# ChristodoulosPappas/IPLS-Java-API

Measured on AMD Instinct MI355X. Metric: aggregated-gradient GB/s (device-resident), 32 peers×4M doubles/partition, higher is better.
Workload: dtype f64

## Files before the change

### ipls-java-api_amd/csrc/engine.hip

```cpp
#include <hip/hip_runtime.h>

#include <algorithm>
#include <atomic>
#include <cstdarg>
#include <cstdio>
#include <cstdlib>
#include <cstring>
#include <deque>
#include <map>
#include <memory>
#include <mutex>
#include <new>
#include <set>
#include <string>
#include <thread>
#include <type_traits>
#include <vector>

#include "../../include/ipls_agg.h"
#include "ipls_kernels.hpp"
#include "javaser.hpp"
#include "engine.hpp"
#include "operand.hpp"
#include "pubsub_host.hpp"
#include "reduce_plan.hpp"

using namespace ipls;
using namespace ipls::reduceplan;
namespace op = ipls::operand;

namespace {

thread_local std::string g_tls_err;

constexpr int64_t kAlignElems = 32;
constexpr int kRingSlots = 4;
constexpr int kStageSlots = 3;

int64_t align_up(int64_t x, int64_t a) { return (x + a - 1) / a * a; }

struct PinnedSlot {
  void* host = nullptr;
  size_t cap = 0;
  hipEvent_t ev = nullptr;
  bool pending = false;
};

}

struct ipls_stage {
  hipStream_t copy[2] = {};
  int n_copy = 0;
  static constexpr int kMaxSlots = 4;
  PinnedSlot slot[kMaxSlots];
  int n_slot = 0;
  void* d = nullptr;
  size_t d_cap = 0;
  hipEvent_t landed[2] = {};
  hipEvent_t ready = nullptr;
  hipEvent_t free_ev = nullptr;
  bool free_pending = false;
};

struct ipls_dev {
  std::mutex mu;
  std::string err;
  int device = 0;
  hipStream_t stream = nullptr;

  int64_t model_size = 0;
  int P = 0;
  int64_t chunk = 0;
  int secure = 0;
  std::vector<int64_t> len, flat_off;
  int64_t max_len = 0, flat_total = 0;
  int p_lo = 0;
  int64_t flat_base = 0;

  double* arena = nullptr;
  int64_t arena_elems = 0;
  std::vector<int64_t> agg_off, rep_off, w_off, fut_off;
  std::vector<uint8_t> agg_zero, rep_zero, fut_zero;

  PinnedSlot ring[kRingSlots];
  void* d_table[kRingSlots] = {};
  size_t d_table_cap[kRingSlots] = {};
  int ring_next = 0;
  std::vector<unsigned char> last_table;
  int last_slot = -1;

  std::mutex stage_mu;
  std::vector<ipls_stage*> stage_all, stage_idle;
  void* d_scratch = nullptr;
  size_t scratch_bytes = 0;
  hipEvent_t copy_ev = nullptr;
  static constexpr int kCopyThreads = 4;
  hipStream_t copy_stream[kCopyThreads] = {};
  hipEvent_t ingest_ev = nullptr;
  std::vector<hipEvent_t> msg_ev;
  struct StageSlot {
    void* d = nullptr;
    size_t cap = 0;
    hipEvent_t free_ev = nullptr;
    bool pending = false;
  };
  StageSlot stage[2];
  int stage_next = 0;
  struct Pending {
    std::vector<const void*> bufs;
    Fmt fmt = kFmtF64;
  };
  std::vector<Pending> pend;
  std::vector<int> pend_keys;
  int pending_n = 0;
  int coalesce = 32;
  struct Batch {
    uint64_t max_ticket;
    hipEvent_t ev;
  };
  static constexpr int kMaxBatches = 64;
  std::deque<Batch> batches;
  std::vector<hipEvent_t> ev_free;
  uint64_t ticket_next = 1, ticket_done = 0, launched_upto = 0;

  unsigned long long* d_sum = nullptr;
  double* d_cnt = nullptr;
  unsigned long long* d_gbuf = nullptr;
  unsigned long long* d_merge = nullptr;
  int64_t merge_cap = 0;
  struct OtherRep {
    unsigned long long* d = nullptr;
    int64_t n = 0;
    int32_t received = 0;
  };
  std::map<std::pair<int, int32_t>, OtherRep> other;
  int64_t gbuf_len = 0;
  ipls_launch_info last_launch{};
};

namespace {

int fail(ipls_dev* h, int code, const char* fmt, ...) {
  char buf[512];
  va_list ap;
  va_start(ap, fmt);
  vsnprintf(buf, sizeof buf, fmt, ap);
  va_end(ap);
  if (h) h->err = buf;
  g_tls_err = buf;
  return code;
}

int not_taken(ipls_dev* h, const op::Refusal& why) { return why.code ? fail(h, why.code, "%s", why.text) : IPLS_OK; }

int flush_pending(ipls_dev* h);

#define IPLS_LOCK(h)                            \
  std::lock_guard<std::mutex> lk_(h->mu);       \
  if (int rc_ = flush_pending(h)) return rc_

#define HIP_TRY(h, expr)                                                                \
  do {                                                                                  \
    hipError_t e_ = (expr);                                                             \
// ... 355 lines not shown
  static constexpr int G = G_, R = R_, MAP = MAP_, BS = BS_, SEQF = SEQF_;
};
template <bool BE_IN, bool BE_OUT, int START, bool FIN = false>
ipls_launch_info launch_reduce_v(int64_t maxL, int n_parts, hipStream_t st, const unsigned long long* const* bufs,
                                 const PartDesc* parts, int k, int secure = 0, const double* cnts = nullptr) {
  constexpr int R = big_r(BE_IN, START), SEQF = big_seqf(BE_IN, START);
  constexpr int RM = mid_r(BE_IN, START), SEQFM = mid_seqf(BE_IN, START);
  const ReducePlan p = plan_reduce(BE_IN, START, FIN, maxL, n_parts);
  const dim3 grid((unsigned)p.grid);
  auto run = [&](auto t) {
    typedef decltype(t) T;
    if constexpr (FIN)
      hipLaunchKernelGGL((k_round<BE_IN, START, T::G, T::R, T::MAP, T::BS, T::SEQF>), grid, dim3(T::BS), 0, st, bufs,
                         parts, k, (int)p.tpp, n_parts, secure, cnts);
    else
      hipLaunchKernelGGL((k_reduce<BE_IN, BE_OUT, START, T::G, T::R, true, T::MAP, T::BS, T::SEQF>), grid,
                         dim3(T::BS), 0, st, bufs, parts, k, (int)p.tpp, n_parts);
  };
  switch (p.shape) {
    case IPLS_SHAPE_HALF:
      if constexpr (half_allowed(START, FIN)) {
        if (p.map == 3) run(Tiles<kBigG, kHalfR, 3, kHalfBS, 0>{});
        else run(Tiles<kBigG, kHalfR, kBigMap, kHalfBS, 0>{});
      }
      break;
    case IPLS_SHAPE_BIG:
      if (p.map == 3) run(Tiles<kBigG, R, 3, kBigBS, SEQF>{});
      else if (p.map == 2) run(Tiles<kBigG, R, 2, kBigBS, SEQF>{});
      else run(Tiles<kBigG, R, kBigMap, kBigBS, SEQF>{});
      break;
    case IPLS_SHAPE_MID:
      if (p.map == 3) run(Tiles<kBigG, RM, 3, kMidBS, SEQFM>{});
      else run(Tiles<kBigG, RM, kBigMap, kMidBS, SEQFM>{});
      break;
    default: run(Tiles<kSmallG, kSmallR, kSmallMap, kSmallBS, 0>{});
  }
  return launch_info(p, BE_IN, BE_OUT, START);
}

ipls_launch_info launch_reduce(bool be_in, bool be_out, int start, int64_t maxL, int n_parts, hipStream_t st,
                               const unsigned long long* const* bufs, const PartDesc* parts, int k) {
  return with_fold(be_in, be_out, start, [&](auto i, auto o, auto s) {
    return launch_reduce_v<decltype(i)::value, decltype(o)::value, decltype(s)::value>(maxL, n_parts, st, bufs, parts, k);
  });
}

ipls_launch_info launch_reduce_fin(bool be_in, int start, int secure, int64_t maxL, int n_parts, hipStream_t st,
                                   const unsigned long long* const* bufs, const PartDesc* parts, int k,
                                   double* cnts) {
  return with_bool(be_in, [&](auto bi) {
    return with_start_za(start, [&](auto s) {
      constexpr bool BI = decltype(bi)::value;
      constexpr int ST = decltype(s)::value;
      hipLaunchKernelGGL((k_round_counts<BI, ST>), dim3(n_parts), dim3(64), 0, st, bufs, parts, k, n_parts, cnts);
      return launch_reduce_v<BI, false, ST, true>(maxL, n_parts, st, bufs, parts, k, secure, cnts);
    });
  });
}

void launch_reduce_scalar(bool be_in, bool be_out, int start, const ReducePlan& p, hipStream_t st,
                          const unsigned long long* const* bufs, const PartDesc* parts, int k) {
  with_fold(be_in, be_out, start, [&](auto bi, auto bo, auto s) {
    hipLaunchKernelGGL((k_reduce_scalar<decltype(bi)::value, decltype(bo)::value, decltype(s)::value>),
                       dim3((unsigned)p.grid), dim3(kBlock), 0, st, bufs, parts, k, (int)p.tpp, p.tile);
  });
}

template <class S>
ipls_launch_info launch_reduce_narrow(bool be_out, int start, bool vec, int64_t maxL, int n_parts, hipStream_t st,
                                      const typename S::elem* const* bufs, const PartDesc* parts, int k) {
  constexpr NarrowShape K = narrow_shape(sizeof(typename S::elem));
  const ReducePlan p = plan_reduce_narrow(sizeof(typename S::elem), false, vec, maxL, n_parts);
  const dim3 grid((unsigned)p.grid);
  with_bool(be_out, [&](auto bo) {
    with_start(start, [&](auto s) {
      auto run = [&](auto map, auto v) {
        constexpr bool V = decltype(v)::value;
        hipLaunchKernelGGL((k_reduce_narrow<S, decltype(bo)::value, decltype(s)::value, K.r, K.bs, decltype(map)::value,
                                            V, (V ? K.pf : 0), K.e>),
                           grid, dim3(K.bs), 0, st, bufs, parts, k, (int)p.tpp, n_parts);
      };
      if (!vec) run(Int<0>{}, std::false_type{});
      else if (p.map == 3) run(Int<3>{}, std::true_type{});
      else run(Int<0>{}, std::true_type{});
    });
  });
  return launch_info(p, false, be_out, start);
}

template <class S, class A>
ipls_launch_info launch_round_narrow(int start, int secure, int64_t maxL, int n_parts, hipStream_t st,
                                     const typename S::elem* const* bufs, const PartDesc* parts, int k,
                                     double* cnts) {
  constexpr NarrowShape K = narrow_shape(sizeof(typename S::elem));
  const ReducePlan p = plan_reduce_narrow(sizeof(typename S::elem), true, true, maxL, n_parts);
  with_start_za(start, [&](auto s) {
    constexpr int ST = decltype(s)::value;
    hipLaunchKernelGGL((k_round_counts_narrow<S, ST>), dim3(n_parts), dim3(64), 0, st, bufs, parts, k, n_parts, cnts);
    hipLaunchKernelGGL((k_round_narrow<S, A, ST, K.r, K.bs, K.pf>), dim3((unsigned)p.grid), dim3(K.bs), 0, st, bufs,
                       parts, k, (int)p.tpp, n_parts, p.map, secure, (const double*)cnts);
  });
  return launch_info(p, false, false, start);
}

struct FinOut {
  unsigned long long* avg;
  Fmt fmt = kFmtF64;
};

constexpr int kFold1NarrowR = 4;
constexpr unsigned kFold1NarrowGrid = 2048;

int reduce_dev(ipls_dev* h, int p_first, int n_parts, const void* const* bufs, int k, Fmt fmt_in,
               int start_mode, int target, void* const* ext_dst = nullptr, bool be_out = false,
               const FinOut* fin = nullptr, bool host_src = false, const int64_t* lens = nullptr,
               bool arrival = false) {
  const bool be_in = fmt_in == kFmtBE, tr_in = fmt_trainer(fmt_in);
  auto len_of = [&](int q) -> int64_t { return lens ? lens[q] : h->len[p_first + q]; };
  auto dst_of = [&](int q) -> unsigned long long* {
    if (fin) return (unsigned long long*)(h->arena + h->w_off[p_first + q]);
    return ext_dst ? (unsigned long long*)ext_dst[q]
                   : (unsigned long long*)(h->arena + target_off(h, p_first + q, target));
  };
  if (k <= 0 && !fin) {
    if (start_mode == IPLS_START_ZERO) {
      for (int q = 0; q < n_parts; ++q) {
        uint8_t* f = ext_dst ? nullptr : zero_flag(h, p_first + q, target);
        if (f) *f = 1;
        else HIP_TRY(h, hipMemsetAsync(dst_of(q), 0, (size_t)len_of(q) * 8, h->stream));
      }
    }
    return IPLS_OK;
  }
  int start = start_mode;
  if (start_mode == IPLS_START_ACCUM && !ext_dst) {
    int nz = 0;
    for (int q = 0; q < n_parts; ++q) {
      uint8_t* f = zero_flag(h, p_first + q, target);
      nz += (f && *f) ? 1 : 0;
    }
    if (nz == n_parts) start = IPLS_START_ZERO;
    else if (nz) {
      for (int q = 0; q < n_parts; ++q) {
        int rc = materialize(h, p_first + q, target);
        if (rc) return rc;
      }
    }
  }
  if (!fin && !tr_in && n_parts == 1 && k == 1 && bufs[0]) {
    unsigned long long* d0 = dst_of(0);
    const int64_t L = len_of(0);
// ... 24 lines not shown
          hipLaunchKernelGGL((k_fold1_narrow<S, decltype(st)::value, kFold1NarrowR>), dim3(blocks), dim3(kBlock), 0,
                             h->stream, d0, s0, L);
        });
      });
      HIP_TRY(h, hipGetLastError());
      h->last_launch = launch_info(fmt_size(fmt_in) == 4 ? IPLS_KERNEL_FOLD1_F32 : IPLS_KERNEL_FOLD1_H16, 0, kBlock,
                                   kFold1NarrowR, 1, 0, blocks, false, false, start);
      if (!ext_dst)
        if (uint8_t* f = zero_flag(h, p_first, target)) *f = 0;
      return IPLS_OK;
    }
  }
  bool aligned16 = true;
  int64_t maxL = 0;
  for (int q = 0; q < n_parts; ++q) maxL = std::max(maxL, len_of(q));
  for (int64_t i = 0; i < (int64_t)n_parts * k; ++i) {
    if (!bufs[i]) return fail(h, IPLS_E_INVAL, "bucket pointer %lld is NULL", (long long)i);
    uintptr_t a = (uintptr_t)bufs[i];
    if (a & (uintptr_t)(fmt_size(fmt_in) - 1))
      return fail(h, IPLS_E_INVAL, "bucket %lld not %d-byte aligned", (long long)i, fmt_size(fmt_in));
    if (a & 15) aligned16 = false;
  }
  const size_t desc_bytes = sizeof(PartDesc) * n_parts;
  const size_t bytes = desc_bytes + sizeof(void*) * (size_t)n_parts * k;
  std::vector<unsigned char> tbl(bytes);
  PartDesc* pd = (PartDesc*)tbl.data();
  for (int q = 0; q < n_parts; ++q) {
    const int p = p_first + q;
    pd[q].len = len_of(q);
    pd[q].dst = dst_of(q);
    pd[q].init = pd[q].dst;
    pd[q].rep = nullptr;
    pd[q].avg = nullptr;
    if (fin) {
      pd[q].init = (const unsigned long long*)(h->arena + h->agg_off[p]);
      if (!h->rep_zero[p]) pd[q].rep = (const unsigned long long*)(h->arena + h->rep_off[p]);
      if (fin->avg)
        pd[q].avg = (unsigned long long*)((char*)fin->avg +
                                          (h->flat_off[p] - h->flat_off[p_first]) * (int64_t)fmt_size(fin->fmt));
    }
    if (!pd[q].dst) return fail(h, IPLS_E_INVAL, "destination %d is NULL", q);
    if ((uintptr_t)pd[q].dst & 7) return fail(h, IPLS_E_INVAL, "destination %d not 8-byte aligned", q);
    if ((uintptr_t)pd[q].dst & 15) aligned16 = false;
  }
  if (k > 0) std::memcpy(tbl.data() + desc_bytes, bufs, sizeof(void*) * (size_t)n_parts * k);
  void* dtab = nullptr;
  int rc = upload_table(h, tbl.data(), bytes, &dtab);
  if (rc) return rc;
  const PartDesc* dparts = (const PartDesc*)dtab;
  auto dbufs = (const unsigned long long* const*)((char*)dtab + desc_bytes);
  if (fin) {
    if (!aligned16 || (fin->avg && tr_in != fmt_trainer(fin->fmt)))
      return fail(h, IPLS_E_INVAL, "fused round needs 16-B aligned buckets and averages of the buckets' family");
    if (tr_in) {
      h->last_launch = with_narrow(fmt_in, [&](auto s) {
        typedef decltype(s) S;
        return with_narrow(fin->avg ? fin->fmt : fmt_in, [&](auto a) {
          return launch_round_narrow<S, decltype(a)>(start, h->secure, maxL, n_parts, h->stream,
                                                     (const typename S::elem* const*)dbufs, dparts, k, h->d_cnt);
        });
      });
    } else {
      h->last_launch = launch_reduce_fin(be_in, start, h->secure, maxL, n_parts, h->stream, dbufs, dparts, k, h->d_cnt);
    }
    HIP_TRY(h, hipGetLastError());
    for (int q = p_first; q < p_first + n_parts; ++q) h->agg_zero[q] = h->rep_zero[q] = 1;
    return IPLS_OK;
  }
  if (tr_in) {
    h->last_launch = with_narrow(fmt_in, [&](auto s) {
      typedef decltype(s) S;
      return launch_reduce_narrow<S>(be_out, start, aligned16, maxL, n_parts, h->stream,
                                     (const typename S::elem* const*)dbufs, dparts, k);
    });
  } else if (aligned16) {
    h->last_launch = launch_reduce(be_in, be_out, start, maxL, n_parts, h->stream, dbufs, dparts, k);
  } else {
    const ReducePlan p = plan_reduce_scalar(maxL, n_parts);
    launch_reduce_scalar(be_in, be_out, start, p, h->stream, dbufs, dparts, k);
    h->last_launch = launch_info(p, be_in, be_out, start);
  }
  HIP_TRY(h, hipGetLastError());
  if (!ext_dst)
    for (int q = 0; q < n_parts; ++q) {
      uint8_t* f = zero_flag(h, p_first + q, target);
      if (f) *f = 0;
    }
  return IPLS_OK;
}

int partition_geometry(const ipls_agg_cfg* c, std::vector<int64_t>& len, std::vector<int64_t>& off,
                       int64_t& chunk, std::string& why) {
  const int P = c->n_partitions;
  len.resize(P);
  off.resize(P);
  if (c->model_size > 0) {
    chunk = ref_chunk(c->model_size, P);
    for (int i = 0; i < P; ++i) {
      int64_t L = ((int64_t)(i + 1) * chunk > c->model_size) ? c->model_size - (int64_t)i * chunk + 1
                                                             : chunk + 1;
      if (L < 1) {
        char b[160];
        snprintf(b, sizeof b, "partition %d length %lld < 1 (%s)", i, (long long)L,
                 L < 0 ? "NegativeArraySizeException, IPLS.java:1863"
                       : "ArrayIndexOutOfBoundsException, IPLS.java:1894");
        why = b;
        return L < 0 ? IPLS_E_NEGSIZE : IPLS_E_RANGE;
      }
      len[i] = L;
      off[i] = (int64_t)i * chunk;
    }
  } else {
    if (c->bucket_len < 1) {
      why = "bucket_len must be >= 1 when model_size == 0";
      return IPLS_E_INVAL;
    }
// ... 159 lines not shown
    lk.lock();
    return fail(h, IPLS_E_DEVICE, "hipStreamSynchronize failed: %s", hipGetErrorString(e));
  }
  return IPLS_OK;
}

int dev_wait(ipls_dev* h, uint64_t ticket) {
  if (!h) return fail(nullptr, IPLS_E_INVAL, "null handle");
  std::unique_lock<std::mutex> lk(h->mu);
  if (ticket >= h->ticket_next) return fail(h, IPLS_E_INVAL, "ticket %llu was never issued", (unsigned long long)ticket);
  if (ticket <= h->ticket_done) return IPLS_OK;
  if (ticket > h->launched_upto)
    if (int rc = flush_pending(h)) return rc;
  hipEvent_t ev = nullptr;
  uint64_t covered = 0;
  for (const auto& b : h->batches)
    if (b.max_ticket >= ticket) {
      ev = b.ev;
      covered = b.max_ticket;
      break;
    }
  if (!ev) return IPLS_OK;
  lk.unlock();
  const hipError_t e = hipEventSynchronize(ev);
  lk.lock();
  if (e != hipSuccess) {
    (void)hipGetLastError();
    return fail(h, IPLS_E_DEVICE, "hipEventSynchronize failed: %s", hipGetErrorString(e));
  }
  while (!h->batches.empty() && h->batches.front().max_ticket <= covered) {
    h->ev_free.push_back(h->batches.front().ev);
    h->batches.pop_front();
  }
  h->ticket_done = std::max(h->ticket_done, covered);
  return IPLS_OK;
}

int dev_flush(ipls_dev* h) {
  if (!h) return fail(nullptr, IPLS_E_INVAL, "null handle");
  IPLS_LOCK(h);
  return IPLS_OK;
}

int dev_set_coalesce(ipls_dev* h, int max_group) {
  if (!h) return fail(nullptr, IPLS_E_INVAL, "null handle");
  IPLS_LOCK(h);
  h->coalesce = std::max(1, max_group);
  return IPLS_OK;
}

namespace {

int end_batch(ipls_dev* h) {
  hipEvent_t ev;
  if (!h->ev_free.empty()) {
    ev = h->ev_free.back();
    h->ev_free.pop_back();
  } else {
    HIP_TRY(h, hipEventCreateWithFlags(&ev, hipEventDisableTiming));
  }
  HIP_TRY(h, hipEventRecord(ev, h->stream));
  h->batches.push_back({h->ticket_next - 1, ev});
  h->launched_upto = h->ticket_next - 1;
  while ((int)h->batches.size() > ipls_dev::kMaxBatches) {
    const ipls_dev::Batch b = h->batches.front();
    HIP_TRY(h, hipEventSynchronize(b.ev));
    h->batches.pop_front();
    h->ev_free.push_back(b.ev);
    h->ticket_done = std::max(h->ticket_done, b.max_ticket);
  }
  return IPLS_OK;
}

int flush_pending(ipls_dev* h) {
  if (h->pend_keys.empty()) return IPLS_OK;
  HIP_TRY(h, dev_use(h->device));
  int rc = IPLS_OK;
  std::vector<int>& keys = h->pend_keys;
  std::sort(keys.begin(), keys.end());
  std::vector<const void*> tab;
  for (size_t i = 0; i < keys.size() && !rc;) {
    const int key = keys[i], target = key / h->P, p0 = key % h->P;
    const ipls_dev::Pending& q0 = h->pend[key];
    const size_t k = q0.bufs.size();
    size_t j = i + 1;
    int n = 1;
    while (j < keys.size() && keys[j] == key + n && keys[j] / h->P == target && h->pend[keys[j]].bufs.size() == k &&
           h->pend[keys[j]].fmt == q0.fmt) {
      ++n;
      ++j;
    }
    tab.clear();
    for (size_t t = i; t < j; ++t) tab.insert(tab.end(), h->pend[keys[t]].bufs.begin(), h->pend[keys[t]].bufs.end());
    rc = reduce_dev(h, p0, n, tab.data(), (int)k, q0.fmt, IPLS_START_ACCUM, target);
    i = j;
  }
  for (int key : keys) h->pend[key].bufs.clear();
  keys.clear();
  h->pending_n = 0;
  if (rc) return rc;
  return end_batch(h);
}

}

int dev_reduce_batch(ipls_dev* h, int p_first, int n_parts, const void* const* bufs, int k,
                          int src_kind, int start_mode, int target) {
  if (!h) return fail(nullptr, IPLS_E_INVAL, "null handle");
  IPLS_LOCK(h);
  if (n_parts <= 0 || p_first < 0 || p_first + n_parts > h->P)
    return fail(h, IPLS_E_RANGE, "partitions [%d,%d) out of range [0,%d)", p_first, p_first + n_parts, h->P);
  if (src_kind != IPLS_DEV_F64 && src_kind != IPLS_DEV_BE && !kind_trainer_dev(src_kind))
    return fail(h, IPLS_E_INVAL, "reduce_batch takes device buckets (DEV_F64/DEV_BE/DEV_F32/DEV_F16/DEV_BF16)");
  if (start_mode < IPLS_START_ACCUM || start_mode > IPLS_START_FIRST) return fail(h, IPLS_E_INVAL, "bad start mode");
  if (target_off(h, 0, target) < 0) return fail(h, IPLS_E_INVAL, "bad target %d", target);
  if (k < 0 || (k > 0 && !bufs)) return fail(h, IPLS_E_INVAL, "bad bucket list");
  HIP_TRY(h, dev_use(h->device));
  return reduce_dev(h, p_first, n_parts, bufs, k, kind_fmt(src_kind), start_mode, target);
}

int dev_accumulate(ipls_dev* h, int p, int target, const void* src, int64_t n, int src_kind) {
  if (!h) return fail(nullptr, IPLS_E_INVAL, "null handle");
  IPLS_LOCK(h);
  if (int rc = check_part(h, p)) return rc;
  if (target_off(h, p, target) < 0) return fail(h, IPLS_E_INVAL, "bad target %d", target);
  const int64_t L = h->len[p];
  op::Resolved v;
  if (op::resolve(op::kAccumulate, src, n, src_kind, L, &v) != op::kTake) return not_taken(h, v.why);
  HIP_TRY(h, dev_use(h->device));
  const size_t bytes = (size_t)L * fmt_size(v.fmt);
  const void* dptr = v.ptr;
  if (v.host) {
    void* alias = nullptr;
    if (v.from == op::kRaw && !fmt_trainer(v.fmt) && op::zero_copy_arrival(v.ptr, bytes) && is_pinned_host(v.ptr, &alias) &&
        alias) {
      const void* bl[1] = {alias};
      if (int rc = reduce_dev(h, p, 1, bl, 1, v.fmt, IPLS_START_ACCUM, target, nullptr, false, nullptr, true)) return rc;
      HIP_TRY(h, hipStreamSynchronize(h->stream));
      return IPLS_OK;
    }
    if (int rc = stage_bucket(h, v.ptr, bytes, &dptr)) return rc;
  }
  const void* bl[1] = {dptr};
  if (int rc = reduce_dev(h, p, 1, bl, 1, v.fmt, IPLS_START_ACCUM, target, nullptr, false, nullptr, false, nullptr,
                          true))
    return rc;
  return v.host ? release_stage(h) : IPLS_OK;
}

int dev_accumulate_async(ipls_dev* h, int p, int target, const void* src, int64_t n, int src_kind,
                              uint64_t* ticket) {
  if (!h || !ticket) return fail(h, IPLS_E_INVAL, "null argument");
  op::Resolved v;
  if (src && (op::kDev & op::bit(src_kind))) {
    std::lock_guard<std::mutex> lk(h->mu);
    if (int rc = check_part(h, p)) return rc;
    if (target_off(h, p, target) < 0) return fail(h, IPLS_E_INVAL, "bad target %d", target);
    if (op::resolve(op::kAccumulateAsync, src, n, src_kind, h->len[p], &v) != op::kTake) return not_taken(h, v.why);
    const Fmt fmt = v.fmt;
    const int qt = target == IPLS_TGT_WADDR ? IPLS_TGT_WEIGHTS : target;
    if (h->pend.empty()) h->pend.resize((size_t)5 * h->P);
    ipls_dev::Pending& q = h->pend[(size_t)qt * h->P + p];
    if (!q.bufs.empty() && q.fmt != fmt)
      if (int rc = flush_pending(h)) return rc;
    if (q.bufs.empty()) h->pend_keys.push_back(qt * h->P + p);
    q.fmt = fmt;
    q.bufs.push_back(src);
    ++h->pending_n;
    *ticket = h->ticket_next++;
    if ((int)q.bufs.size() >= 2 * h->coalesce || h->pending_n >= h->coalesce * (int)h->pend_keys.size())
      return flush_pending(h);
    return IPLS_OK;
  }
  void* alias = nullptr;
  const bool host = op::kHostD & op::bit(src_kind);
  if (!src || !host || !op::zero_copy_queued(src) || !is_pinned_host(src, &alias) || !alias) {
    int rc = dev_accumulate(h, p, target, src, n, src_kind);
    std::lock_guard<std::mutex> lk(h->mu);
    *ticket = h->ticket_done;
    return rc;
  }
  IPLS_LOCK(h);
  if (int rc = check_part(h, p)) return rc;
  if (target_off(h, p, target) < 0) return fail(h, IPLS_E_INVAL, "bad target %d", target);
  if (op::resolve(op::kAccumulateAsync, src, n, src_kind, h->len[p], &v) != op::kTake) return not_taken(h, v.why);
  HIP_TRY(h, dev_use(h->device));
  const void* bl[1] = {alias};
  if (int rc = reduce_dev(h, p, 1, bl, 1, v.fmt, IPLS_START_ACCUM, target, nullptr, false, nullptr, true)) return rc;
  *ticket = h->ticket_next++;
  return end_batch(h);
}

int dev_accumulate_range(ipls_dev* h, int p, int target, const void* src, int64_t off, int64_t n, int src_kind,
                         uint64_t* ticket) {
  if (!h || !ticket || !src) return fail(h, IPLS_E_INVAL, "null argument");
  IPLS_LOCK(h);
  if (int rc = check_part(h, p)) return rc;
  if (target_off(h, p, target) < 0) return fail(h, IPLS_E_INVAL, "bad target %d", target);
  const int64_t L = h->len[p];
  op::Resolved v;
  if (op::resolve(op::kAccumulateRange, src, n, src_kind, L, &v) != op::kTake) return not_taken(h, v.why);
  if (off < 0 || n < 0 || off > L || n > L - off)
    return fail(h, IPLS_E_RANGE, "range [%lld, %lld) outside partition %d of length %lld", (long long)off,
                (long long)(off + n), p, (long long)L);
  if ((off & 1) || !op::zero_copy_queued(src))
    return fail(h, IPLS_E_INVAL, "a ranged fold needs an even start and 16-B aligned bytes");
  void* alias = nullptr;
  if (!is_pinned_host(src, &alias) || !alias)
    return fail(h, IPLS_E_INVAL, "a ranged fold reads pinned host memory (ipls_host_alloc)");
  if (n == 0) {
    *ticket = h->ticket_done;
    return IPLS_OK;
  }
  HIP_TRY(h, dev_use(h->device));
  if (int rc = materialize(h, p, target)) return rc;
  unsigned long long* d0 = (unsigned long long*)(h->arena + target_off(h, p, target)) + off;
  const auto* s0 = (const unsigned long long*)alias;
  const unsigned blocks = std::max(1u, std::min<unsigned>(blocks_for(n >> 1, kBlock * 4), 128u));
// ... 510 lines not shown
                       (const FinDesc*)dtab, h->arena, tpp);
  HIP_TRY(h, hipGetLastError());
  for (int q = p0; q < p0 + np; ++q) h->agg_zero[q] = h->rep_zero[q] = 1;
  return IPLS_OK;
}

static int divide_table(ipls_dev* h, int p0, int np, const DivDesc** dtab, int* tpp) {
  std::vector<DivDesc> dd(np);
  int64_t maxn = 0;
  for (int q = 0; q < np; ++q) {
    const int p = p0 + q;
    dd[q] = DivDesc{h->len[p], h->w_off[p], h->flat_off[p] - h->flat_off[p0]};
    maxn = std::max(maxn, h->len[p] - 1);
  }
  *tpp = (int)((std::max<int64_t>(maxn, 0) + kDivTile - 1) / kDivTile);
  if (*tpp == 0) return IPLS_OK;
  void* d = nullptr;
  if (int rc = upload_table(h, dd.data(), dd.size() * sizeof(DivDesc), &d)) return rc;
  *dtab = (const DivDesc*)d;
  return IPLS_OK;
}

static int divide_range(ipls_dev* h, int p0, int np, unsigned long long* d_out, bool be) {
  const DivDesc* dtab = nullptr;
  int tpp = 0;
  if (int rc = divide_table(h, p0, np, &dtab, &tpp)) return rc;
  if (tpp == 0) return IPLS_OK;
  with_bool(be, [&](auto b) {
    with_bool(h->secure != 0, [&](auto sec) {
      hipLaunchKernelGGL((k_divide<decltype(b)::value, decltype(sec)::value>), dim3((unsigned)tpp * np), dim3(kBlock),
                         0, h->stream, dtab, (const double*)h->arena, d_out, tpp);
    });
  });
  HIP_TRY(h, hipGetLastError());
  return IPLS_OK;
}

static int divide_range_narrow(ipls_dev* h, int p0, int np, void* d_out, Fmt fmt) {
  const DivDesc* dtab = nullptr;
  int tpp = 0;
  if (int rc = divide_table(h, p0, np, &dtab, &tpp)) return rc;
  if (tpp == 0) return IPLS_OK;
  with_narrow(fmt, [&](auto s) {
    typedef decltype(s) S;
    with_bool(h->secure != 0, [&](auto sec) {
      hipLaunchKernelGGL((k_divide_narrow<S, decltype(sec)::value>), dim3((unsigned)tpp * np), dim3(kBlock), 0,
                         h->stream, dtab, (const double*)h->arena, (typename S::elem*)d_out, tpp);
    });
  });
  HIP_TRY(h, hipGetLastError());
  return IPLS_OK;
}

int dev_finalize(ipls_dev* h, int p, void* sum_out, int sum_kind, double* avg_out) {
  if (!h) return fail(nullptr, IPLS_E_INVAL, "null handle");
  IPLS_LOCK(h);
  int p0 = p, np = 1;
  if (p == IPLS_ALL_PARTITIONS) {
    p0 = 0;
    np = h->P;
    if (sum_out || avg_out) return fail(h, IPLS_E_INVAL, "host outputs need a single partition");
  } else if (int rc = check_part(h, p)) {
    return rc;
  }
  if (sum_out && sum_kind != IPLS_HOST_F64 && sum_kind != IPLS_HOST_BE)
    return fail(h, IPLS_E_INVAL, "sum_kind must be HOST_F64 or HOST_BE");
  HIP_TRY(h, dev_use(h->device));
  if (int rc = finalize_range(h, p0, np)) return rc;

  if (np == 1 && (sum_out || avg_out)) {
    const int64_t L = h->len[p0];
    const double* w = h->arena + h->w_off[p0];
    if (sum_out) {
      if (sum_kind == IPLS_HOST_F64) {
        if (int rc = d2h(h, sum_out, w, (size_t)L * 8)) return rc;
      } else if (sum_kind == IPLS_HOST_BE) {
        if (int rc = be_to_host(h, sum_out, w, L)) return rc;
      } else {
        return fail(h, IPLS_E_INVAL, "sum_kind must be HOST_F64 or HOST_BE");
      }
    }
    if (avg_out && L > 1) {
      if (int rc = ensure_scratch(h, (size_t)L * 8)) return rc;
      if (int rc = divide_range(h, p0, 1, (unsigned long long*)h->d_scratch, false)) return rc;
      if (int rc = d2h(h, avg_out, h->d_scratch, (size_t)(L - 1) * 8)) return rc;
    }
  }
  return IPLS_OK;
}

int dev_finalize_chunked(ipls_dev* h, int p, int sum_kind, int64_t chunk, ipls_chunk_sink sink, void* ctx) {
  if (!h || !sink) return fail_nl(h, IPLS_E_INVAL, "null argument");
  if (chunk < 2 || (chunk & 1))
    return fail_nl(h, IPLS_E_INVAL, "chunk of %lld values: even and >= 2", (long long)chunk);
  if (p < 0 || p >= h->P) return fail_nl(h, IPLS_E_RANGE, "partition %d out of range [0,%d)", p, h->P);
  if (sum_kind != IPLS_HOST_F64 && sum_kind != IPLS_HOST_BE)
    return fail_nl(h, IPLS_E_INVAL, "sum_kind must be HOST_F64 or HOST_BE");
  const int64_t L = h->len[p];
  HIP_TRY_NL(h, dev_use(h->device));
  const int64_t c = std::min(chunk, L);
  ipls_stage* st = nullptr;
  if (int rc = stage_acquire(h, (size_t)L * 8, (size_t)c * 8, &st)) return rc;
  int rc = IPLS_OK;
  {
    std::lock_guard<std::mutex> lk(h->mu);
    rc = flush_pending(h);
    if (!rc) rc = finalize_range(h, p, 1);
    if (!rc) {
      const unsigned long long* w = (const unsigned long long*)(h->arena + h->w_off[p]);
      hipError_t e;
      if (sum_kind == IPLS_HOST_BE) {
        launch_bswap(h->stream, w, (unsigned long long*)st->d, L);
        e = hipGetLastError();
      } else {
        e = hipMemcpyAsync(st->d, w, (size_t)L * 8, hipMemcpyDeviceToDevice, h->stream);
      }
      if (e == hipSuccess) e = hipEventRecord(st->ready, h->stream);
      if (e != hipSuccess) {
        (void)hipGetLastError();
        rc = fail(h, IPLS_E_DEVICE, "W snapshot: %s", hipGetErrorString(e));
      }
    }
  }
  if (rc) {
    (void)hipStreamSynchronize(h->stream);
    (void)hipGetLastError();
    stage_release(h, st);
    return rc;
  }
  return stage_deliver(h, st, L, c, 0, sink, ctx, " (the round is consumed)");
}

int dev_set_weights(ipls_dev* h, int p, const void* src, int64_t n, int src_kind) {
  if (!h || !src) return fail(h, IPLS_E_INVAL, "null argument");
  IPLS_LOCK(h);
  if (int rc = check_part(h, p)) return rc;
  const int64_t L = h->len[p];
  op::Resolved v;
  if (op::resolve(op::kSetWeights, src, n, src_kind, L, &v) != op::kTake) return not_taken(h, v.why);
  HIP_TRY(h, dev_use(h->device));
  const int64_t m = v.from == op::kFrame ? L : v.n;
  double* w = h->arena + h->w_off[p];
  const void* d = v.ptr;
  if (v.host) {
    if (v.fmt == kFmtF64) return stage_h2d(h, w, v.ptr, (size_t)m * 8);
    if (int rc = to_scratch(h, v.ptr, (size_t)m * 8)) return rc;
    d = h->d_scratch;
  } else if (v.fmt == kFmtF64) {
    HIP_TRY(h, hipMemcpyAsync(w, v.ptr, (size_t)m * 8, hipMemcpyDeviceToDevice, h->stream));
    return IPLS_OK;
  }
  launch_bswap(h->stream, (const unsigned long long*)d, (unsigned long long*)w, m);
  HIP_TRY(h, hipGetLastError());
  return IPLS_OK;
}

static int flat_to_device(ipls_dev* h, const op::SrcView& v, const unsigned long long** d) {
  *d = (const unsigned long long*)v.ptr;
  if (!v.host) return IPLS_OK;
  if (int rc = to_scratch(h, v.ptr, (size_t)v.n * fmt_size(v.fmt))) return rc;
// ... 380 lines not shown
  hipError_t e = hipGetLastError();
  if (e != hipSuccess) return fail(nullptr, IPLS_E_DEVICE, "k_synth launch: %s", hipGetErrorString(e));
  return IPLS_OK;
}

int ipls_checksum_dev(const void* src, int64_t n, int src_kind, uint64_t* out, void* stream) {
  if (!out || n < 0 || (n > 0 && !src)) return fail(nullptr, IPLS_E_INVAL, "bad argument");
  if (n == 0) {
    *out = 0;
    return IPLS_OK;
  }
  hipStream_t st = (hipStream_t)stream;
  unsigned long long* d = nullptr;
  if (hipMallocAsync((void**)&d, 8, st) != hipSuccess) {
    (void)hipGetLastError();
    return fail(nullptr, IPLS_E_NOMEM, "hipMallocAsync failed");
  }
  hipMemsetAsync(d, 0, 8, st);
  const dim3 g(std::max(1u, std::min<unsigned>(blocks_for(n, kBlock * 8), 2048)));
  if (src_kind == IPLS_DEV_BE)
    hipLaunchKernelGGL(k_checksum<true>, g, dim3(kBlock), 0, st, (const unsigned long long*)src, n, d);
  else
    hipLaunchKernelGGL(k_checksum<false>, g, dim3(kBlock), 0, st, (const unsigned long long*)src, n, d);
  unsigned long long v = 0;
  hipError_t e = hipGetLastError();
  if (e == hipSuccess) e = hipMemcpyAsync(&v, d, 8, hipMemcpyDeviceToHost, st);
  if (e == hipSuccess) e = hipStreamSynchronize(st);
  hipFreeAsync(d, st);
  if (e != hipSuccess) return fail(nullptr, IPLS_E_DEVICE, "checksum: %s", hipGetErrorString(e));
  *out = v;
  return IPLS_OK;
}

int dev_reduce_batch_out(ipls_dev* h, int p_first, int n_parts, const void* const* bufs, int k, int src_kind,
                              int start_mode, void* const* dst, int dst_kind) {
  if (!h) return fail(nullptr, IPLS_E_INVAL, "null handle");
  IPLS_LOCK(h);
  if (n_parts <= 0 || p_first < 0 || p_first + n_parts > h->P)
    return fail(h, IPLS_E_RANGE, "partitions [%d,%d) out of range [0,%d)", p_first, p_first + n_parts, h->P);
  if (src_kind != IPLS_DEV_F64 && src_kind != IPLS_DEV_BE && !kind_trainer_dev(src_kind))
    return fail(h, IPLS_E_INVAL, "reduce_batch_out takes device buckets (DEV_F64/DEV_BE/DEV_F32/DEV_F16/DEV_BF16)");
  if (dst_kind != IPLS_DEV_F64 && dst_kind != IPLS_DEV_BE)
    return fail(h, IPLS_E_INVAL, "reduce_batch_out writes device buffers (DEV_F64/DEV_BE)");
  if (start_mode < IPLS_START_ACCUM || start_mode > IPLS_START_FIRST) return fail(h, IPLS_E_INVAL, "bad start mode");
  if (!dst || k < 0 || (k > 0 && !bufs)) return fail(h, IPLS_E_INVAL, "bad bucket/destination list");
  HIP_TRY(h, dev_use(h->device));
  return reduce_dev(h, p_first, n_parts, bufs, k, kind_fmt(src_kind), start_mode, IPLS_TGT_AGG, dst,
                    dst_kind == IPLS_DEV_BE);
}

int dev_aggregate_round(ipls_dev* h, int p_first, int n_parts, const void* const* bufs, int k, int src_kind,
                             void* avg_out, int avg_kind) {
  if (!h) return fail(nullptr, IPLS_E_INVAL, "null handle");
  IPLS_LOCK(h);
  if (n_parts <= 0 || p_first < 0 || p_first + n_parts > h->P)
    return fail(h, IPLS_E_RANGE, "partitions [%d,%d) out of range [0,%d)", p_first, p_first + n_parts, h->P);
  if (src_kind != IPLS_DEV_F64 && src_kind != IPLS_DEV_BE && !kind_trainer_dev(src_kind))
    return fail(h, IPLS_E_INVAL, "aggregate_round takes device buckets (DEV_F64/DEV_BE/DEV_F32/DEV_F16/DEV_BF16)");
  const Fmt fmt_in = kind_fmt(src_kind);
  const bool tr_in = fmt_trainer(fmt_in);
  const bool tr_avg = avg_out && kind_trainer(avg_kind);
  const Fmt fmt_avg = tr_avg ? kind_fmt(avg_kind) : kFmtF64;
  if (avg_out && !tr_avg && avg_kind != IPLS_DEV_F64 && avg_kind != IPLS_HOST_F64)
    return fail(h, IPLS_E_INVAL, "avg_kind must be DEV_F64, HOST_F64 or a DEV/HOST F32, F16 or BF16 kind");
  if (k < 0 || (k > 0 && !bufs)) return fail(h, IPLS_E_INVAL, "bad bucket list");
  if (tr_in)
    for (int64_t i = 0; i < (int64_t)n_parts * k; ++i)
      if (!bufs[i] || ((uintptr_t)bufs[i] & (uintptr_t)(fmt_size(fmt_in) - 1)))
        return fail(h, IPLS_E_INVAL, "bucket %lld NULL or not %d-byte aligned", (long long)i, fmt_size(fmt_in));
  HIP_TRY(h, dev_use(h->device));
  const int p_last = p_first + n_parts - 1;
  const int64_t n_avg = h->flat_off[p_last] + h->len[p_last] - 1 - h->flat_off[p_first];
  unsigned long long* d_avg = nullptr;
  if (tr_avg && n_avg > 0) {
    if ((uintptr_t)avg_out & (uintptr_t)(fmt_size(fmt_avg) - 1))
      return fail(h, IPLS_E_INVAL, "output not %d-byte aligned", fmt_size(fmt_avg));
    if (kind_trainer_dev(avg_kind)) {
      d_avg = (unsigned long long*)avg_out;
    } else {
      if (int rc = ensure_scratch(h, (size_t)n_avg * fmt_size(fmt_avg))) return rc;
      d_avg = (unsigned long long*)h->d_scratch;
    }
  } else if (avg_out && n_avg > 0) {
    if (avg_kind == IPLS_DEV_F64) {
      if ((uintptr_t)avg_out & 7) return fail(h, IPLS_E_INVAL, "device output not 8-byte aligned");
      d_avg = (unsigned long long*)avg_out;
    } else {
      if (int rc = ensure_scratch(h, (size_t)n_avg * 8)) return rc;
      d_avg = (unsigned long long*)h->d_scratch;
    }
  }
  bool aligned16 = true;
  for (int64_t i = 0; i < (int64_t)n_parts * k; ++i) aligned16 = aligned16 && !((uintptr_t)bufs[i] & 15);
  if (aligned16 && (tr_in ? (!avg_out || tr_avg) : !tr_avg)) {
    FinOut fo{d_avg, fmt_avg};
    if (int rc = reduce_dev(h, p_first, n_parts, bufs, k, fmt_in, IPLS_START_ACCUM, IPLS_TGT_AGG,
                            nullptr, false, &fo))
      return rc;
  } else {
    if (int rc = reduce_dev(h, p_first, n_parts, bufs, k, fmt_in, IPLS_START_ACCUM, IPLS_TGT_AGG)) return rc;
    if (int rc = finalize_range(h, p_first, n_parts)) return rc;
    if (d_avg) {
      if (tr_avg) {
        if (int rc = divide_range_narrow(h, p_first, n_parts, d_avg, fmt_avg)) return rc;
      } else if (int rc = divide_range(h, p_first, n_parts, d_avg, false)) {
        return rc;
      }
    }
  }
  if (d_avg && kind_trainer_host(avg_kind)) return d2h(h, avg_out, d_avg, (size_t)n_avg * fmt_size(fmt_avg));
  if (d_avg && avg_kind == IPLS_HOST_F64) return d2h(h, avg_out, d_avg, (size_t)n_avg * 8);
  return IPLS_OK;
}

namespace {

int ingest_copy_threads() {
  static const int n = [] {
    const char* e = std::getenv("IPLS_INGEST_COPY_THREADS");
    const int v = e ? std::atoi(e) : 2;
    return std::max(1, std::min(v, (int)ipls_dev::kCopyThreads));
  }();
  return n;
}

}

int dev_ingest_pubsub(ipls_dev* h, int target, const uint8_t* const* msgs, const int64_t* lens, int n_msgs,
                           int layers, const int32_t* parts, int32_t* status) {
  if (!h) return fail(nullptr, IPLS_E_INVAL, "null handle");
  IPLS_LOCK(h);
  if (n_msgs < 0 || (n_msgs > 0 && (!msgs || !lens))) return fail(h, IPLS_E_INVAL, "bad message list");
  if (layers < 1 || layers > 2) return fail(h, IPLS_E_INVAL, "layers must be 1 or 2");
  if (target_off(h, 0, target) < 0) return fail(h, IPLS_E_INVAL, "bad target %d", target);
  if (n_msgs == 0) return 0;
  HIP_TRY(h, dev_use(h->device));

  std::vector<int32_t> st(n_msgs, 0), post(n_msgs, 0), route(n_msgs, -1);
  std::vector<int64_t> dc(n_msgs, 0), dc2(n_msgs, 0);
  std::vector<uint8_t> decode(n_msgs, 0);
  for (int i = 0; i < n_msgs; ++i) {
    const pubsub::Pre pre = pubsub::precheck(msgs[i], lens[i], layers);
    if (pre.status) { st[i] = pre.status; continue; }
    dc[i] = pre.dc;
    dc2[i] = pre.dc2;
    decode[i] = 1;
    if (pre.n == 0) { post[i] = 1; continue; }
// ... 894 lines not shown
```

Before: 7139.

## Fuse pending queue fold into finalize round and skip count kernel when unused

Adds a close_range path that folds only the pending queues for the target partitions and, when buffers are aligned, runs them through the fused reduce-plus-finalize-plus-average kernel. Finalize no longer needs separate flush, finalize and divide passes. Ticket accounting now tracks per-queue first tickets so that partial flushes only mark completed work as launched. The count kernel is skipped when no average is requested. This adds complexity to batch and ticket bookkeeping, and dev_aggregate_round now flushes the pending queues first when given explicit buckets.

```diff
diff --git a/ipls-java-api_amd/csrc/engine.hip b/ipls-java-api_amd/csrc/engine.hip
--- a/ipls-java-api_amd/csrc/engine.hip
+++ b/ipls-java-api_amd/csrc/engine.hip
@@ -24,6 +24,7 @@
 #include "operand.hpp"
 #include "pubsub_host.hpp"
 #include "reduce_plan.hpp"
+#include "ticket_rule.hpp"
 
 using namespace ipls;
 using namespace ipls::reduceplan;
@@ -109,6 +110,7 @@
   struct Pending {
     std::vector<const void*> bufs;
     Fmt fmt = kFmtF64;
+    uint64_t first_ticket = 0;
   };
   std::vector<Pending> pend;
   std::vector<int> pend_keys;
@@ -570,7 +572,8 @@
     return with_start_za(start, [&](auto s) {
       constexpr bool BI = decltype(bi)::value;
       constexpr int ST = decltype(s)::value;
-      hipLaunchKernelGGL((k_round_counts<BI, ST>), dim3(n_parts), dim3(64), 0, st, bufs, parts, k, n_parts, cnts);
+      if (cnts)
+        hipLaunchKernelGGL((k_round_counts<BI, ST>), dim3(n_parts), dim3(64), 0, st, bufs, parts, k, n_parts, cnts);
       return launch_reduce_v<BI, false, ST, true>(maxL, n_parts, st, bufs, parts, k, secure, cnts);
     });
   });
@@ -614,7 +617,8 @@
   const ReducePlan p = plan_reduce_narrow(sizeof(typename S::elem), true, true, maxL, n_parts);
   with_start_za(start, [&](auto s) {
     constexpr int ST = decltype(s)::value;
-    hipLaunchKernelGGL((k_round_counts_narrow<S, ST>), dim3(n_parts), dim3(64), 0, st, bufs, parts, k, n_parts, cnts);
+    if (cnts)
+      hipLaunchKernelGGL((k_round_counts_narrow<S, ST>), dim3(n_parts), dim3(64), 0, st, bufs, parts, k, n_parts, cnts);
     hipLaunchKernelGGL((k_round_narrow<S, A, ST, K.r, K.bs, K.pf>), dim3((unsigned)p.grid), dim3(K.bs), 0, st, bufs,
                        parts, k, (int)p.tpp, n_parts, p.map, secure, (const double*)cnts);
   });
@@ -745,16 +749,17 @@
   if (fin) {
     if (!aligned16 || (fin->avg && tr_in != fmt_trainer(fin->fmt)))
       return fail(h, IPLS_E_INVAL, "fused round needs 16-B aligned buckets and averages of the buckets' family");
+    double* const cnts = fin->avg ? h->d_cnt : nullptr;
     if (tr_in) {
       h->last_launch = with_narrow(fmt_in, [&](auto s) {
         typedef decltype(s) S;
         return with_narrow(fin->avg ? fin->fmt : fmt_in, [&](auto a) {
           return launch_round_narrow<S, decltype(a)>(start, h->secure, maxL, n_parts, h->stream,
-                                                     (const typename S::elem* const*)dbufs, dparts, k, h->d_cnt);
+                                                     (const typename S::elem* const*)dbufs, dparts, k, cnts);
         });
       });
     } else {
-      h->last_launch = launch_reduce_fin(be_in, start, h->secure, maxL, n_parts, h->stream, dbufs, dparts, k, h->d_cnt);
+      h->last_launch = launch_reduce_fin(be_in, start, h->secure, maxL, n_parts, h->stream, dbufs, dparts, k, cnts);
     }
     HIP_TRY(h, hipGetLastError());
     for (int q = p_first; q < p_first + n_parts; ++q) h->agg_zero[q] = h->rep_zero[q] = 1;
@@ -1020,6 +1025,10 @@
 namespace {
 
 int end_batch(ipls_dev* h) {
+  std::vector<uint64_t> first_queued;
+  for (int key : h->pend_keys) first_queued.push_back(h->pend[key].first_ticket);
+  const uint64_t upto = tickets::launched_upto(h->ticket_next, first_queued.data(), first_queued.size());
+  if (upto == h->launched_upto) return IPLS_OK;
   hipEvent_t ev;
   if (!h->ev_free.empty()) {
     ev = h->ev_free.back();
@@ -1028,8 +1037,8 @@
     HIP_TRY(h, hipEventCreateWithFlags(&ev, hipEventDisableTiming));
   }
   HIP_TRY(h, hipEventRecord(ev, h->stream));
-  h->batches.push_back({h->ticket_next - 1, ev});
-  h->launched_upto = h->ticket_next - 1;
+  h->batches.push_back({upto, ev});
+  h->launched_upto = upto;
   while ((int)h->batches.size() > ipls_dev::kMaxBatches) {
     const ipls_dev::Batch b = h->batches.front();
     HIP_TRY(h, hipEventSynchronize(b.ev));
@@ -1040,20 +1049,17 @@
   return IPLS_OK;
 }
 
-int flush_pending(ipls_dev* h) {
-  if (h->pend_keys.empty()) return IPLS_OK;
-  HIP_TRY(h, dev_use(h->device));
+int fold_queues(ipls_dev* h, const std::vector<int>& keys, size_t i, size_t end) {
   int rc = IPLS_OK;
-  std::vector<int>& keys = h->pend_keys;
-  std::sort(keys.begin(), keys.end());
   std::vector<const void*> tab;
-  for (size_t i = 0; i < keys.size() && !rc;) {
+  const size_t first = i;
+  while (i < end && !rc) {
     const int key = keys[i], target = key / h->P, p0 = key % h->P;
     const ipls_dev::Pending& q0 = h->pend[key];
     const size_t k = q0.bufs.size();
     size_t j = i + 1;
     int n = 1;
-    while (j < keys.size() && keys[j] == key + n && keys[j] / h->P == target && h->pend[keys[j]].bufs.size() == k &&
+    while (j < end && keys[j] == key + n && keys[j] / h->P == target && h->pend[keys[j]].bufs.size() == k &&
            h->pend[keys[j]].fmt == q0.fmt) {
       ++n;
       ++j;
@@ -1063,9 +1069,21 @@
     rc = reduce_dev(h, p0, n, tab.data(), (int)k, q0.fmt, IPLS_START_ACCUM, target);
     i = j;
   }
-  for (int key : keys) h->pend[key].bufs.clear();
+  for (size_t t = first; t < end; ++t) {
+    ipls_dev::Pending& q = h->pend[keys[t]];
+    h->pending_n -= (int)q.bufs.size();
+    q.bufs.clear();
+  }
+  return rc;
+}
+
+int flush_pending(ipls_dev* h) {
+  if (h->pend_keys.empty()) return IPLS_OK;
+  HIP_TRY(h, dev_use(h->device));
+  std::vector<int>& keys = h->pend_keys;
+  std::sort(keys.begin(), keys.end());
+  const int rc = fold_queues(h, keys, 0, keys.size());
   keys.clear();
-  h->pending_n = 0;
   if (rc) return rc;
   return end_batch(h);
 }
@@ -1131,7 +1149,10 @@
     ipls_dev::Pending& q = h->pend[(size_t)qt * h->P + p];
     if (!q.bufs.empty() && q.fmt != fmt)
       if (int rc = flush_pending(h)) return rc;
-    if (q.bufs.empty()) h->pend_keys.push_back(qt * h->P + p);
+    if (q.bufs.empty()) {
+      h->pend_keys.push_back(qt * h->P + p);
+      q.first_ticket = h->ticket_next;
+    }
     q.fmt = fmt;
     q.bufs.push_back(src);
     ++h->pending_n;
@@ -1748,9 +1769,95 @@
   return IPLS_OK;
 }
 
+static int close_range(ipls_dev* h, int p0, int np, const FinOut* fo, Fmt fmt_empty = kFmtF64) {
+  HIP_TRY(h, dev_use(h->device));
+  std::vector<int>& keys = h->pend_keys;
+  std::sort(keys.begin(), keys.end());
+  const int a0 = IPLS_TGT_AGG * h->P;
+  auto part_of = [&](int key) {
+    if (key < a0 || key >= a0 + h->P) return 0;
+    return key >= a0 + p0 && key < a0 + p0 + np ? 1 : 2;
+  };
+  std::stable_sort(keys.begin(), keys.end(), [&](int a, int b) { return part_of(a) < part_of(b); });
+  size_t n_other = 0, n_in = 0;
+  for (int key : keys) {
+    n_other += part_of(key) == 0;
+    n_in += part_of(key) == 1;
+  }
+  auto launched = [&](size_t n) {
+    keys.erase(keys.begin(), keys.begin() + n);
+    return end_batch(h);
+  };
+  if (n_other) {
+    const int rc = fold_queues(h, keys, 0, n_other);
+    const int rb = launched(n_other);
+    if (rc || rb) return rc ? rc : rb;
+  }
+  auto queue_of = [&](int p) -> const ipls_dev::Pending* {
+    if (h->pend.empty()) return nullptr;
+    const ipls_dev::Pending& q = h->pend[(size_t)a0 + p];
+    return q.bufs.empty() ? nullptr : &q;
+  };
+  const bool want_avg = fo && fo->avg;
+  auto fusable = [&](int p) {
+    const ipls_dev::Pending* q = queue_of(p);
+    if (!q && !fo) return false;
+    if (q)
+      for (const void* b : q->bufs)
+        if ((uintptr_t)b & 15) return false;
+    return !want_avg || fmt_trainer(q ? q->fmt : fmt_empty) == fmt_trainer(fo->fmt);
+  };
+  bool all_fusable = true;
+  for (int p = p0; p < p0 + np; ++p) all_fusable = all_fusable && fusable(p);
+  if (want_avg && !all_fusable) {
+    const int rc = n_in ? fold_queues(h, keys, 0, n_in) : IPLS_OK;
+    const int rb = n_in ? launched(n_in) : IPLS_OK;
+    if (rc || rb) return rc ? rc : rb;
+    if (int rc2 = finalize_range(h, p0, np)) return rc2;
+    return fmt_trainer(fo->fmt) ? divide_range_narrow(h, p0, np, fo->avg, fo->fmt) : divide_range(h, p0, np, fo->avg, false);
+  }
+  std::vector<const void*> tab;
+  for (int p = p0; p < p0 + np;) {
+    const bool fused = all_fusable || fusable(p);
+    const ipls_dev::Pending* q0 = queue_of(p);
+    const size_t k = q0 ? q0->bufs.size() : 0;
+    const Fmt fmt = q0 ? q0->fmt : fmt_empty;
+    int e = p + 1;
+    size_t nk = q0 ? 1 : 0;
+    for (; e < p0 + np; ++e) {
+      const ipls_dev::Pending* q = queue_of(e);
+      if (fused ? !(fusable(e) && (q ? q->bufs.size() : 0) == k && (q ? q->fmt : fmt_empty) == fmt) : fusable(e)) break;
+      nk += q ? 1 : 0;
+    }
+    int rc;
+    if (fused) {
+      tab.clear();
+      if (k)
+        for (int t = p; t < e; ++t) tab.insert(tab.end(), h->pend[(size_t)a0 + t].bufs.begin(), h->pend[(size_t)a0 + t].bufs.end());
+      const FinOut run{want_avg ? (unsigned long long*)((char*)fo->avg + (h->flat_off[p] - h->flat_off[p0]) *
+                                                                           (int64_t)fmt_size(fo->fmt))
+                                : nullptr,
+                       fo ? fo->fmt : kFmtF64};
+      rc = reduce_dev(h, p, e - p, tab.data(), (int)k, fmt, IPLS_START_ACCUM, IPLS_TGT_AGG, nullptr, false, &run);
+      for (size_t t = 0; t < nk; ++t) {
+        ipls_dev::Pending& q = h->pend[keys[t]];
+        h->pending_n -= (int)q.bufs.size();
+        q.bufs.clear();
+      }
+    } else {
+      rc = nk ? fold_queues(h, keys, 0, nk) : IPLS_OK;
+      if (!rc) rc = finalize_range(h, p, e - p);
+    }
+    const int rb = nk ? launched(nk) : IPLS_OK;
+    if (rc || rb) return rc ? rc : rb;
+    p = e;
+  }
+  return IPLS_OK;
+}
+
 int dev_finalize(ipls_dev* h, int p, void* sum_out, int sum_kind, double* avg_out) {
   if (!h) return fail(nullptr, IPLS_E_INVAL, "null handle");
-  IPLS_LOCK(h);
+  std::lock_guard<std::mutex> lk_(h->mu);
   int p0 = p, np = 1;
   if (p == IPLS_ALL_PARTITIONS) {
     p0 = 0;
@@ -1761,8 +1868,7 @@
   }
   if (sum_out && sum_kind != IPLS_HOST_F64 && sum_kind != IPLS_HOST_BE)
     return fail(h, IPLS_E_INVAL, "sum_kind must be HOST_F64 or HOST_BE");
-  HIP_TRY(h, dev_use(h->device));
-  if (int rc = finalize_range(h, p0, np)) return rc;
+  if (int rc = close_range(h, p0, np, nullptr)) return rc;
 
   if (np == 1 && (sum_out || avg_out)) {
     const int64_t L = h->len[p0];
@@ -1800,8 +1906,7 @@
   int rc = IPLS_OK;
   {
     std::lock_guard<std::mutex> lk(h->mu);
-    rc = flush_pending(h);
-    if (!rc) rc = finalize_range(h, p, 1);
+    rc = close_range(h, p, 1, nullptr);
     if (!rc) {
       const unsigned long long* w = (const unsigned long long*)(h->arena + h->w_off[p]);
       hipError_t e;
@@ -2288,7 +2393,9 @@
 int dev_aggregate_round(ipls_dev* h, int p_first, int n_parts, const void* const* bufs, int k, int src_kind,
                              void* avg_out, int avg_kind) {
   if (!h) return fail(nullptr, IPLS_E_INVAL, "null handle");
-  IPLS_LOCK(h);
+  std::lock_guard<std::mutex> lk_(h->mu);
+  if (k != 0)
+    if (int rc = flush_pending(h)) return rc;
   if (n_parts <= 0 || p_first < 0 || p_first + n_parts > h->P)
     return fail(h, IPLS_E_RANGE, "partitions [%d,%d) out of range [0,%d)", p_first, p_first + n_parts, h->P);
   if (src_kind != IPLS_DEV_F64 && src_kind != IPLS_DEV_BE && !kind_trainer_dev(src_kind))
@@ -2328,7 +2435,10 @@
   }
   bool aligned16 = true;
   for (int64_t i = 0; i < (int64_t)n_parts * k; ++i) aligned16 = aligned16 && !((uintptr_t)bufs[i] & 15);
-  if (aligned16 && (tr_in ? (!avg_out || tr_avg) : !tr_avg)) {
+  if (k == 0) {
+    const FinOut fo{d_avg, fmt_avg};
+    if (int rc = close_range(h, p_first, n_parts, &fo, fmt_in)) return rc;
+  } else if (aligned16 && (tr_in ? (!avg_out || tr_avg) : !tr_avg)) {
     FinOut fo{d_avg, fmt_avg};
     if (int rc = reduce_dev(h, p_first, n_parts, bufs, k, fmt_in, IPLS_START_ACCUM, IPLS_TGT_AGG,
                             nullptr, false, &fo))
diff --git a/ipls-java-api_amd/csrc/ticket_rule.hpp b/ipls-java-api_amd/csrc/ticket_rule.hpp
--- /dev/null
+++ b/ipls-java-api_amd/csrc/ticket_rule.hpp
@@ -0,0 +1,16 @@
+#pragma once
+#include <cstddef>
+#include <cstdint>
+
+namespace ipls {
+namespace tickets {
+
+inline uint64_t launched_upto(uint64_t ticket_next, const uint64_t* first_queued, size_t n) {
+  uint64_t upto = ticket_next - 1;
+  for (size_t i = 0; i < n; ++i)
+    if (first_queued[i] - 1 < upto) upto = first_queued[i] - 1;
+  return upto;
+}
+
+}
+}
```

Measured after the change: 7022. 1.6% lower.
